# fortio/tray

Measured on AMD Instinct MI355X. Metric: Mrays/sec, seed-2 book-cover scene 1280x720 r=64 d=50; per-pixel L∞ vs ref, higher is better.
Workload: dtype f64; 1 GPU; C2 book-cover seed 2 1280x720 r=64 d=50; traversal=bvh, width=1280, height=720, rays_per_pixel=64, max_depth=50, scene_seed=2, spheres=486, output=float3 f32 linear, parallelism=row-tiles x1, tile_rows=0, frames_in_flight=2, frames_per_launch=16

## Files before the change

tray_amd/csrc/rng.hpp:

```cpp
#pragma once

#include <hip/hip_runtime.h>
#include <stdint.h>

namespace tray {

enum : uint32_t { kPurposeCamera = 1, kPurposeScatter = 3, kPurposeScene = 4, kPurposeKey = 5 };

struct U2 {
    double u0, u1;
};
struct U4 {
    double u0, u1, u2, u3;
};

struct Block {
    uint32_t x0, x1, x2, x3;
};

#ifndef TRAY_PHILOX_ROUNDS
#define TRAY_PHILOX_ROUNDS 10
#endif
__host__ __device__ __forceinline__ Block philox4x32_10(uint64_t seed, uint32_t c0, uint32_t c1, uint32_t c2,
                                                        uint32_t c3) {
    uint32_t k0 = (uint32_t)seed, k1 = (uint32_t)(seed >> 32);
#pragma unroll
    for (int r = 0; r < TRAY_PHILOX_ROUNDS; ++r) {
        if (r > 0) {
            k0 += 0x9E3779B9u;
            k1 += 0xBB67AE85u;
        }
        const uint64_t p0 = (uint64_t)0xD2511F53u * c0;
        const uint64_t p1 = (uint64_t)0xCD9E8D57u * c2;
        const uint32_t n0 = (uint32_t)(p1 >> 32) ^ c1 ^ k0;
        const uint32_t n2 = (uint32_t)(p0 >> 32) ^ c3 ^ k1;
        c0 = n0;
        c1 = (uint32_t)p1;
        c2 = n2;
        c3 = (uint32_t)p0;
    }
    return Block{c0, c1, c2, c3};
}

struct DrawKey {
    uint32_t k0, k1, k2, k3;
};
__host__ __device__ inline DrawKey draw_key(uint64_t seed) {
    const Block b = philox4x32_10(seed, 0u, 0u, 0u, kPurposeKey << 24);
    return DrawKey{b.x0, b.x1, b.x2, b.x3};
}

__host__ __device__ __forceinline__ Block draw_block(uint32_t k0, uint32_t k1, uint32_t k2, uint32_t k3, uint32_t pixel,
                                                     uint32_t sample, uint32_t bounce, uint32_t purpose) {
    uint32_t v0 = (pixel ^ k0) * 1664525u + 1013904223u, v1 = (sample ^ k1) * 1664525u + 1013904223u;
    uint32_t v2 = (bounce ^ k2) * 1664525u + 1013904223u, v3 = (purpose ^ k3) * 1664525u + 1013904223u;
    v0 += v1 * v3;
    v1 += v2 * v0;
    v2 += v0 * v1;
    v3 += v1 * v2;
    v0 ^= v0 >> 16;
    v1 ^= v1 >> 16;
    v2 ^= v2 >> 16;
    v3 ^= v3 >> 16;
    v0 += v1 * v3;
    v1 += v2 * v0;
    v2 += v0 * v1;
    v3 += v1 * v2;
    return Block{v0 ^ (v0 >> 16), v1 ^ (v1 >> 16), v2 ^ (v2 >> 16), v3 ^ (v3 >> 16)};
}

__host__ __device__ __forceinline__ U2 philox_uniforms(uint64_t seed, uint32_t c0, uint32_t c1, uint32_t c2,
                                                       uint32_t c3) {
    const Block b = philox4x32_10(seed, c0, c1, c2, c3);
    const uint64_t a = ((uint64_t)b.x1 << 32) | b.x0;
    const uint64_t c = ((uint64_t)b.x3 << 32) | b.x2;
    U2 u;
    u.u0 = (double)(a >> 11) * 0x1.0p-53;
    u.u1 = (double)(c >> 11) * 0x1.0p-53;
    return u;
}

__host__ __device__ __forceinline__ void sincos_2pi(double u, double& s, double& c) {
    const double v = u * 4.0;
    const double q = __builtin_floor(v);
    const double f = v - q;
    const int quad = (int)q;
    const bool swap = f > 0.5;
    const float x = (float)(swap ? 1.0 - f : f);
    const float t = x * 0x1.921fb6p+0f;
    const float t2 = t * t;
    float sp = __builtin_fmaf(t2, 0x1.71de3ap-19f, -0x1.a01a02p-13f);
    sp = __builtin_fmaf(sp, t2, 0x1.111112p-7f);
    sp = __builtin_fmaf(sp, t2, -0x1.555556p-3f);
    sp = __builtin_fmaf(sp, t2, 1.0f);
    float sn = t * sp;
    float cp = __builtin_fmaf(t2, -0x1.27e4fcp-22f, 0x1.a01a02p-16f);
    cp = __builtin_fmaf(cp, t2, -0x1.6c16c2p-10f);
    cp = __builtin_fmaf(cp, t2, 0x1.555556p-5f);
    cp = __builtin_fmaf(cp, t2, -0.5f);
    float cs = __builtin_fmaf(cp, t2, 1.0f);
    if (swap) {
        const float tmp = sn;
        sn = cs;
        cs = tmp;
    }
    const double sd = sn, cd = cs;
    const double k = 1.5 - 0.5 * (sd * sd + cd * cd);
    const double sk = sd * k, ck = cd * k;
    const int qq = quad & 3;
    s = qq == 0 ? sk : qq == 1 ? ck : qq == 2 ? -sk : -ck;
    c = qq == 0 ? ck : qq == 1 ? -sk : qq == 2 ? -ck : sk;
}

__host__ __device__ __forceinline__ void sincos_2pi_word(uint32_t w, double& s, double& c) {
    const uint32_t F = w & 0x3FFFFFFFu;
    const bool swap = F > 0x20000000u;
    const float x = (float)(swap ? 0x40000000u - F : F) * 0x1p-30f;
    const float t = x * 0x1.921fb6p+0f;
    const float t2 = t * t;
    float sp = __builtin_fmaf(t2, 0x1.71de3ap-19f, -0x1.a01a02p-13f);
    sp = __builtin_fmaf(sp, t2, 0x1.111112p-7f);
    sp = __builtin_fmaf(sp, t2, -0x1.555556p-3f);
    sp = __builtin_fmaf(sp, t2, 1.0f);
    float sn = t * sp;
    float cp = __builtin_fmaf(t2, -0x1.27e4fcp-22f, 0x1.a01a02p-16f);
    cp = __builtin_fmaf(cp, t2, -0x1.6c16c2p-10f);
    cp = __builtin_fmaf(cp, t2, 0x1.555556p-5f);
    cp = __builtin_fmaf(cp, t2, -0.5f);
    float cs = __builtin_fmaf(cp, t2, 1.0f);
    if (swap) {
        const float tmp = sn;
        sn = cs;
        cs = tmp;
    }
    const double sd = sn, cd = cs;
    const double k = 1.5 - 0.5 * (sd * sd + cd * cd);
    const double sk = sd * k, ck = cd * k;
    const uint32_t qq = w >> 30;
    const bool swap_sc = (qq & 1u) != 0u;
    const double s0 = swap_sc ? ck : sk, c0 = swap_sc ? sk : ck;
    const uint64_t sflip = (uint64_t)(qq >> 1) << 63, cflip = (uint64_t)((qq ^ (qq >> 1)) & 1u) << 63;
    s = __builtin_bit_cast(double, __builtin_bit_cast(uint64_t, s0) ^ sflip);
    c = __builtin_bit_cast(double, __builtin_bit_cast(uint64_t, c0) ^ cflip);
}

}
```

tray_amd/csrc/tray_kernel.hip:

```cpp

#include <hip/hip_runtime.h>
#include <stdint.h>
#include <stdlib.h>

#include <algorithm>

#include "bvh.hpp"
#include "fp64.hpp"
#include "rng.hpp"
#include "tray_internal.hpp"
#include "tray_kernel.hpp"

namespace tray {

struct D3 {
    double x, y, z;
};

__device__ __forceinline__ D3 d3(double x, double y, double z) { return D3{x, y, z}; }
__device__ __forceinline__ D3 add(D3 u, D3 v) { return d3(v.x + u.x, v.y + u.y, v.z + u.z); }
__device__ __forceinline__ D3 sub(D3 u, D3 v) { return d3(u.x - v.x, u.y - v.y, u.z - v.z); }
__device__ __forceinline__ D3 smul(D3 v, double t) { return d3(v.x * t, v.y * t, v.z * t); }
__device__ __forceinline__ D3 mul(D3 u, D3 v) { return d3(u.x * v.x, u.y * v.y, u.z * v.z); }
__device__ __forceinline__ D3 sdiv(D3 v, double t) { return d3(v.x / t, v.y / t, v.z / t); }
// ... 532 lines not shown
#define TRAY_WAVE_CHUNKS 32
#endif
#ifndef TRAY_LATE_TAKES
#define TRAY_LATE_TAKES 8u
#endif
__device__ __forceinline__ uint32_t take_chunk(const KernelParams& p, UniPtr uni, uint32_t lane, uint32_t G,
                                               uint32_t& count) {
    typedef __attribute__((address_space(3))) uint64_t LdsU64;
    LdsU64* pool = (LdsU64*)&uni->pool;
    const volatile __attribute__((address_space(3))) uint32_t* pool_end =
        (const volatile __attribute__((address_space(3))) uint32_t*)&uni->pool + 1;
    while (true) {
        uint64_t old = 0;
        if (lane == 0) old = __hip_atomic_fetch_add(pool, (uint64_t)G, __ATOMIC_RELAXED, __HIP_MEMORY_SCOPE_WORKGROUP);
        const uint32_t next = __builtin_amdgcn_readlane((uint32_t)old, 0);
        const uint32_t end = __builtin_amdgcn_readlane((uint32_t)(old >> 32), 0);
        if (end == kPoolDone) return kPoolDone;
        if (next + G <= end) {
            count = G;
            return next;
        }
        if (next <= end) {
            uint32_t base = 0;
            const uint32_t pool_chunks = __builtin_amdgcn_readfirstlane(uni->pool_chunks);
            if (lane == 0) base = atomicAdd(p.queue, pool_chunks);
            base = __builtin_amdgcn_readlane(base, 0);
            const uint64_t fresh = base >= p.nchunks
                                       ? (uint64_t)kPoolDone << 32
                                       : ((uint64_t)min(base + pool_chunks, p.nchunks) << 32) | base;
            if (lane == 0) __hip_atomic_store(pool, fresh, __ATOMIC_RELAXED, __HIP_MEMORY_SCOPE_WORKGROUP);
            if (next < end) {
                count = end - next;
                return next;
            }
            continue;
        }
        while (__builtin_amdgcn_readlane(*pool_end, 0) == end) __builtin_amdgcn_s_sleep(1);
    }
}

__device__ __forceinline__ bool decode_item(const KernelParams& p, uint32_t i, uint32_t tile, int32_t& x, int32_t& j,
                                            uint32_t& s, uint32_t& k) {
    k = 0;
    uint32_t q = udiv(i, p.div_spp, s);
    if (p.passes > 1) q = udiv(q, p.div_passes, k);
    const uint32_t r = q & 63u;
    if (!p.tile_order) tile = q >> 6;
    uint32_t tx;
    const uint32_t ty = udiv(tile, p.div_tiles_x, tx);
    x = (int32_t)(tx * 8u + (r & 7u));
    const int32_t jb = (int32_t)(ty * 8u + (r >> 3));
    j = p.j0 + jb;
    return x < p.width && jb < p.band_rows;
}
__device__ __forceinline__ uint32_t chunk_tile(const KernelParams& p, uint32_t c) {
    if (!p.tile_order) return 0u;
    uint32_t rem;
    return __builtin_amdgcn_readfirstlane(p.tile_order[udiv(c, p.div_chunks_per_tile, rem)]);
}

__device__ __forceinline__ void start_sample(const KernelParams& p, Lane& L, uint32_t item, int32_t x,
                                             int32_t j, uint32_t s) {
    const int32_t y = row_of(p, j);
    L.item = item;
    L.x = x;
    L.j = j;
    L.pixel = (uint32_t)y * (uint32_t)p.width + (uint32_t)x;
    L.sample = s;
    L.bounce = 0;
    L.segments = 0;
    L.thr = d3(1, 1, 1);
    L.busy = true;
    get_ray(p, camera_block(p, L.pixel, s), (double)x, (double)y, L.org, L.dir);
}

template <bool kStats, int kAcc>
__device__ __forceinline__ void end_path(const KernelParams& p, Lane& L, const D3& color, Stats& st,
                                         const AccCtx& acc) {
    if constexpr (kAcc) {
#ifdef TRAY_PROBE_NO_ACC_ADD
        if (color.x != 12345.0) return void(L.busy = false);
#endif
        const uint32_t rs = acc_rshift<kAcc>(p);
        const uint32_t group = ((L.slot << (6u - rs)) | ((L.item & 63u) >> rs));
        LdsF64* s = acc.slabs + (group * kAccCopies + (threadIdx.x % kAccCopies)) * 3u;
        __hip_atomic_fetch_add(s + 0, __builtin_rint(color.x), __ATOMIC_RELAXED, __HIP_MEMORY_SCOPE_WAVEFRONT);
        __hip_atomic_fetch_add(s + 1, __builtin_rint(color.y), __ATOMIC_RELAXED, __HIP_MEMORY_SCOPE_WAVEFRONT);
        __hip_atomic_fetch_add(s + 2, __builtin_rint(color.z), __ATOMIC_RELAXED, __HIP_MEMORY_SCOPE_WAVEFRONT);
#ifdef TRAY_WO_LINEAR_COST
        if (p.tile_cost)
            __hip_atomic_fetch_add(acc.counts + L.slot, L.segments, __ATOMIC_RELAXED, __HIP_MEMORY_SCOPE_WAVEFRONT);
#else
        if (p.tile_cost)
            __hip_atomic_fetch_add(acc.counts + L.slot, L.segments * L.segments, __ATOMIC_RELAXED,
                                   __HIP_MEMORY_SCOPE_WAVEFRONT);
#endif
    } else {
        double* o = p.samples + (size_t)L.item * 3;
        o[0] = color.x;
        o[1] = color.y;
        o[2] = color.z;
    }
    if (p.segments) atomicAdd(p.segments + (size_t)L.j * (size_t)p.width + (size_t)L.x, L.segments);
    if constexpr (kStats) st.segments += L.segments;
    L.busy = false;
}

__device__ __forceinline__ void flush_progress(const KernelParams& p, int32_t t, uint64_t n, uint32_t lane) {
    if (n != 0u && lane == 0u)
        __hip_atomic_fetch_add(p.progress + t, (unsigned long long)n, __ATOMIC_RELAXED, __HIP_MEMORY_SCOPE_SYSTEM);
}
__device__ __forceinline__ void count_progress(const KernelParams& p, bool ended, int32_t j, uint32_t lane,
                                               int32_t& cur, uint64_t& cnt) {
    uint64_t m = __ballot(ended);
    while (m != 0ull) {
        const uint32_t first = (uint32_t)__builtin_ctzll(m);
        const int32_t t0 = __builtin_amdgcn_readlane(j >> 3, first);
        const uint64_t same = __ballot(ended && (j >> 3) == t0) & m;
        if (t0 != cur) {
            flush_progress(p, cur, cnt, lane);
            cur = t0;
            cnt = 0u;
        }
        cnt += (uint64_t)__popcll(same);
        m &= ~same;
    }
}

template <int kFmt>
__device__ __forceinline__ void write_pixel(const KernelParams& p, const double* srgb, D3 mean, int32_t x, int32_t j,
                                            uint32_t pass) {
    const size_t off = (size_t)j * (size_t)p.width + (size_t)x;
    void* const out = static_cast<char*>(p.out) + (size_t)pass * p.out_frame_bytes;
    if constexpr (kFmt == kOutRGBF64) {
        double* o = static_cast<double*>(out) + off * 3;
        o[0] = mean.x;
        o[1] = mean.y;
        o[2] = mean.z;
    } else if constexpr (kFmt == kOutRGBF32) {
        float* o = static_cast<float*>(out) + off * 3;
        o[0] = (float)mean.x;
        o[1] = (float)mean.y;
        o[2] = (float)mean.z;
    } else {
        static_cast<uint32_t*>(out)[off] = srgba_word(srgb, mean.x, mean.y, mean.z);
    }
}
template <int kFmt>
__device__ __forceinline__ void write_mean(const KernelParams& p, const double* srgb, D3 sum, int32_t x, int32_t j,
                                           uint32_t pass) {
    const double inv = 1.0 / (double)p.spp;
    const D3 mean = smul(sum, inv);
    write_pixel<kFmt>(p, srgb, mean, x, j, pass);
}

template <int kAcc>
__device__ __forceinline__ uint64_t acc_retire(const KernelParams& p, const AccCtx& acc, uint64_t open, bool busy,
                                               uint32_t slot, uint32_t chunk_of, uint32_t lane) {
    uint64_t freed = 0;
    while (open != 0ull) {
        const uint32_t s0 = (uint32_t)__builtin_ctzll(open);
        open &= open - 1ull;
        if (__ballot(busy && slot == s0) == 0ull) freed |= 1ull << s0;
    }
    if ((freed >> lane) & 1ull) {
        const uint32_t groups = 64u >> acc_rshift<kAcc>(p);
        uint32_t count = 0u;
        if (p.tile_cost) {
            volatile LdsU32* n = acc.counts;
            count = n[lane];
            n[lane] = 0u;
        }
        for (uint32_t g = 0; g < groups; ++g) {
            const uint32_t slab = kAcc == 1 ? lane : lane * groups + g;
            volatile LdsF64* v = acc.slabs + slab * kAccCopies * 3u;
            double sum[3] = {0.0, 0.0, 0.0};
#pragma unroll
            for (int k = 0; k < kAccCopies; ++k)
#pragma unroll
                for (int c = 0; c < 3; ++c) sum[c] += v[3 * k + c];
#pragma unroll
            for (int k = 0; k < 3 * kAccCopies; ++k) v[k] = 0.0;
            AccPartial* o = reinterpret_cast<AccPartial*>(p.samples) + (kAcc == 1 ? chunk_of : chunk_of * groups + g);
            o->sum[0] = sum[0];
            o->sum[1] = sum[1];
            o->sum[2] = sum[2];
            o->pad = g == 0 ? (double)count : 0.0;
            if constexpr (kAcc == 1) break;
        }
    }
    return freed;
}



template <bool kWild>
__device__ __forceinline__ bool shade_end_color(const KernelParams& p, const Lane& L, bool hit, double dir_lsq,
                                                D3& color) {
    const bool last = L.bounce + 1u >= (uint32_t)p.max_depth;
    const bool blind = kWild ? false : last;
    if (hit && !blind) return true;
    color = d3(0, 0, 0);
    if (!hit) {
        const D3 ud = unit_lsq(L.dir, dir_lsq);
        const double t = 0.5 * (ud.y + 1.0);
        const D3 bg_a = d3(p.bg_a.x, p.bg_a.y, p.bg_a.z), bg_b = d3(p.bg_b.x, p.bg_b.y, p.bg_b.z);
        color = mul(L.thr, add(smul(bg_a, 1.0 - t), smul(bg_b, t)));
    }
    return false;
}
template <bool kStats, int kAcc, bool kWild>
__device__ __forceinline__ bool shade_end(const KernelParams& p, Lane& L, bool hit, double dir_lsq, Stats& st,
                                          const AccCtx& acc) {
    D3 color;
    if (shade_end_color<kWild>(p, L, hit, dir_lsq, color)) return true;
    end_path<kStats, kAcc>(p, L, color, st, acc);
    return false;
}

template <bool kWild, typename GeoAt, typename MatAt>
__device__ __forceinline__ bool shade_scatter_color(const KernelParams& p, Lane& L, double closest, double dir_lsq,
                                                    GeoAt geo_at, MatAt mat_at, D3& color) {
    const double4 g = geo_at();
    const MatRec m = mat_at();
    const Block w = draw(p, L.pixel, L.sample, L.bounce, kPurposeScatter);
    const double u0 = uniform(w.x0);
    D3 ud = d3(0, 0, 0);
    if (m.type != kLambertian) ud = unit_lsq(L.dir, dir_lsq);
    color = d3(0, 0, 0);
    bool ends = false;
    {
        const D3 point = add(L.org, smul(L.dir, closest));
        const D3 outward = sdiv_rcp(sub(point, d3(g.x, g.y, g.z)), m.radius, m.rinv);
        const bool front = dot(L.dir, outward) < 0;
        const D3 normal = neg_if(outward, !front);
        bool scattered = true;
        D3 new_dir;
        D3 att = d3(m.albedo[0], m.albedo[1], m.albedo[2]);
        const bool lambertian = m.type == kLambertian, dielectric = m.type == kDielectric;
        const double cos_theta = go_min1(dot(neg(ud), normal));
        const double z = 1.0 - 2.0 * u0;
        const double sq = sqrt_cr(dielectric ? 1.0 - cos_theta * cos_theta : 1.0 - z * z);
        D3 uv = d3(0, 0, 0);
        if (lambertian || (m.type == kMetal && m.param > 0.0)) uv = unit_vector_from(z, sq, w.x1);
        if (lambertian) {
            new_dir = add(normal, uv);
            if (near_zero(new_dir)) new_dir = normal;
        } else if (m.type == kMetal) {
            D3 reflected = reflect(ud, normal);
            if (m.param > 0.0) reflected = add(reflected, smul(uv, m.param));
            new_dir = reflected;
            scattered = dot(new_dir, normal) > 0;
        } else {
            att = d3(1.0, 1.0, 1.0);
            const double ratio = front ? m.pinv : m.param;
            const double sin_theta = sq;
            const double r0 = front ? m.albedo[0] : m.albedo[1];
            const bool do_reflect = ratio * sin_theta > 1.0 || reflectance(cos_theta, r0) > u0;
            new_dir = do_reflect ? reflect(ud, normal) : refract(ud, normal, ratio);
        }
        if (scattered && (kWild ? L.bounce + 1u < (uint32_t)p.max_depth : true)) {
            L.thr = mul(L.thr, att);
            L.org = point;
            L.dir = new_dir;
            ++L.bounce;
        } else {
            ends = true;
            if constexpr (kWild) color = smul(scattered ? mul(L.thr, att) : L.thr, 0.0);
        }
    }
    __builtin_amdgcn_s_waitcnt(0x0F70);
    return !ends;
}
template <bool kStats, int kAcc, bool kWild, typename GeoAt, typename MatAt>
__device__ __forceinline__ bool shade_scatter(const KernelParams& p, Lane& L, double closest, double dir_lsq,
                                              GeoAt geo_at, MatAt mat_at, Stats& st, const AccCtx& acc) {
    D3 color;
    if (shade_scatter_color<kWild>(p, L, closest, dir_lsq, geo_at, mat_at, color)) return true;
    end_path<kStats, kAcc>(p, L, color, st, acc);
    return false;
}

template <bool kStats, int kAcc, bool kWild, typename GeoAt, typename MatAt>
__device__ __forceinline__ bool shade_step(const KernelParams& p, Lane& L, int best, double closest,
                                           double dir_lsq, GeoAt geo_at, MatAt mat_at, Stats& st, const AccCtx& acc) {
    D3 color;
    bool goes_on = false;
    if (shade_end_color<kWild>(p, L, best >= 0, dir_lsq, color))
        goes_on = shade_scatter_color<kWild>(p, L, closest, dir_lsq, geo_at, mat_at, color);
    if (goes_on) return true;
    end_path<kStats, kAcc>(p, L, color, st, acc);
    return false;
}

#ifndef TRAY_DEVICE_FUNCTIONS_ONLY

#ifndef TRAY_WAVES_PER_SIMD
#define TRAY_WAVES_PER_SIMD 5
#endif
#ifndef TRAY_NODE_STEPS
#define TRAY_NODE_STEPS 3
#endif
#ifndef TRAY_NODE_STEPS_MAX
#define TRAY_NODE_STEPS_MAX 5
#endif
constexpr int kDeepSteps = TRAY_NODE_STEPS_MAX + 1;
// ... 27 lines not shown
            asm volatile("v_add_f32_e64 %0, 1.0, 1.0" : "=v"(t_));            \
        }                                                                     \
    }
#define TRAY_PROBE_F64(n)                                                     \
    {                                                                         \
        _Pragma("unroll") for (int i_ = 0; i_ < (n); ++i_) {                  \
            double t_;                                                        \
            asm volatile("v_add_f64 %0, 1.0, 1.0" : "=v"(t_));                \
        }                                                                     \
    }

#ifdef TRAY_CENSUS
#define TRAY_MARK(name) asm volatile(";@phase " name);
#else
#define TRAY_MARK(name)
#endif

#ifdef TRAY_PROFILE
#define PROF_T0() const uint64_t prof_t0_ = __builtin_amdgcn_s_memtime()
#define PROF_ADD(slot) PROF_CNT(slot, __builtin_amdgcn_s_memtime() - prof_t0_)
#define PROF_CNT(slot, v)                                  \
    {                                                      \
        const unsigned long long v_ = (v);                 \
        if (lane == 0) atomicAdd(prof + (slot), v_);       \
    }
#define PROF_T0E() PROF_T0()
#define PROF_ADDE(slot) PROF_ADD(slot)
#elif defined(TRAY_PROFILE_TIMELINE)
#define PROF_T0() const uint64_t prof_t0_ = (kStats && tl_lone) ? __builtin_amdgcn_s_memtime() : 0
#define PROF_ADD(slot) \
    if (kStats && tl_lone) tl_ph[slot] += __builtin_amdgcn_s_memtime() - prof_t0_
#define PROF_CNT(slot, v)
#else
#define PROF_T0()
#define PROF_ADD(slot)
#define PROF_CNT(slot, v)
#endif
#ifndef TRAY_PROFILE
#define PROF_T0E()
#define PROF_ADDE(slot)
#endif

#if defined(TRAY_PROFILE_BEGIN) && (defined(TRAY_PROFILE_REFILL) || defined(TRAY_PROFILE_CANDWAIT))
#error "TRAY_PROFILE_BEGIN shares profile slots with TRAY_PROFILE_REFILL / TRAY_PROFILE_CANDWAIT"
#endif
#ifdef TRAY_PROFILE_MATERIAL
constexpr int kMatCounters = 26;
__device__ __forceinline__ void prof_material(int site, bool active, int32_t slot, uint32_t bounce, int32_t max_depth,
                                              const MatRec* bmat, uint32_t lane, unsigned long long* pm) {
    int cls = -1;
    if (active) {
        if (slot < 0) cls = 0;
        else if (bounce + 1u >= (uint32_t)max_depth) cls = 1;
        else {
            const MatRec& m = bmat[slot];
            cls = m.type == kLambertian ? 2 : m.type == kDielectric ? 5 : m.param > 0.0 ? 4 : 3;
        }
    }
    unsigned long long* c = pm + site * kMatCounters;
    int bodies = 0;
    for (int k = 0; k < 6; ++k) {
        const uint64_t m = __ballot(cls == k);
        if (lane == 0 && m) {
            atomicAdd(c + k, 1ull);
            atomicAdd(c + 6 + k, (unsigned long long)__popcll(m));
        }
    }
    bodies = (__ballot(cls == 2) ? 1 : 0) + (__ballot(cls == 3 || cls == 4) ? 1 : 0) + (__ballot(cls == 5) ? 1 : 0);
    const int n_di = __popcll(__ballot(cls == 5)), n_me = __popcll(__ballot(cls == 3 || cls == 4));
    const int n_active = __popcll(__ballot(active));
    if (lane == 0) {
        if (n_di) atomicAdd(c + 18 + (n_di >= 8 ? 3 : n_di >= 4 ? 2 : n_di >= 2 ? 1 : 0), 1ull);
        if (n_me) atomicAdd(c + 22 + (n_me >= 8 ? 3 : n_me >= 4 ? 2 : n_me >= 2 ? 1 : 0), 1ull);
        atomicAdd(c + 12 + bodies, 1ull);
        atomicAdd(c + 16, 1ull);
        atomicAdd(c + 17, (unsigned long long)n_active);
    }
}
#define PROF_MATERIAL(site, active) prof_material(site, active, T.slot, L.bounce, p.max_depth, p.bmat, lane, prof_mat)
#else
#define PROF_MATERIAL(site, active)
#endif

#ifdef TRAY_PROFILE_TIMELINE
constexpr uint32_t kTlBuckets = 1024, kTlTicks = 25000, kTlHdr = 6, kTlStride = kTlBuckets + kTlHdr;
#endif

__device__ __forceinline__ uint64_t wave_sum_u64(uint64_t v) {
#pragma unroll
    for (int off = 32; off >= 1; off >>= 1) v += __shfl_xor(v, off, 64);
    return v;
}


__host__ __device__ constexpr size_t bvh_stack_bytes(int32_t slots) { return (size_t)slots * kStackSlotBytes; }

template <int kLDS, bool kBVH, bool kStats, bool kSpill, bool kProg, int kAcc, int kSteps = TRAY_NODE_STEPS_MAX,
          bool kWild = false>
__global__ __launch_bounds__(kBVH ? kBvhBlock : 256, kBVH ? TRAY_BVH_WAVES_PER_SIMD : TRAY_WAVES_PER_SIMD) void render_kernel(KernelParams p) {
    static_assert(!(kWild && (kBVH || kAcc != 0)), "kWild: linear scan, FP64 sums");
    extern __shared__ __attribute__((aligned(16))) double4 smem_all[];
    __attribute__((address_space(3))) Uniforms* uni_lds =
        (__attribute__((address_space(3))) Uniforms*)reinterpret_cast<Uniforms*>(smem_all);
    double4* smem = smem_all + kUniformsBytes / sizeof(double4);
    if (threadIdx.x == 0) {
        volatile __attribute__((address_space(3))) Uniforms* u = uni_lds;
        u->pool = 0;
        u->pool_chunks = p.pool_chunks;
    }
    const UniPtr uni = uni_lds;
    SceneView sv{p.geo,  p.nodes, p.leaves,    p.leaf_single != 0,       p.bgeo, p.bidx,
                 p.bmat, p.n,     p.n_nodes,   p.n_global, p.n_slots - p.n_global};
    Stack<kSpill> S{nullptr, nullptr, 0, 0};
    if constexpr (kBVH) {
        S.base = (__attribute__((address_space(3))) uint32_t*)reinterpret_cast<uint32_t*>(smem) + threadIdx.x;
        S.lds = p.stack_lds;
        S.stride = gridDim.x * blockDim.x;
        if constexpr (kSpill) S.ovf = p.stack_ovf + blockIdx.x * blockDim.x + threadIdx.x;
        double4* scene = smem + bvh_stack_bytes(p.stack_lds) / sizeof(double4);
        if constexpr (kLDS == 1) {
            double4* lds_nodes = scene;
            double4* lds_geo = scene + (size_t)p.n_nodes * (sizeof(Bvh4Node) / sizeof(double4));
            int32_t* lds_idx = reinterpret_cast<int32_t*>(lds_geo + p.n_slots);
            int32_t* lds_leaves = lds_idx + p.n_slots;
            const double4* gn = reinterpret_cast<const double4*>(p.nodes);
            const int n4 = p.n_nodes * (int)(sizeof(Bvh4Node) / sizeof(double4));
            for (int i = threadIdx.x; i < n4; i += blockDim.x) lds_nodes[i] = gn[i];
            for (int i = threadIdx.x; i < p.n_slots; i += blockDim.x) {
                lds_geo[i] = p.bgeo[i];
                lds_idx[i] = p.bidx[i];
            }
            for (int i = threadIdx.x; i < p.n_leaves; i += blockDim.x) lds_leaves[i] = p.leaves[i];
            sv.nodes = reinterpret_cast<const Bvh4Node*>(lds_nodes);
            sv.bgeo = lds_geo;
            sv.bidx = lds_idx;
            sv.leaves = lds_leaves;
        } else if constexpr (kLDS == 2) {
            double4* lds_nodes = scene;
            int32_t* lds_leaves =
                reinterpret_cast<int32_t*>(scene + (size_t)p.n_nodes * (sizeof(Bvh4Node) / sizeof(double4)));
            const double4* gn = reinterpret_cast<const double4*>(p.nodes);
            const int n4 = p.n_nodes * (int)(sizeof(Bvh4Node) / sizeof(double4));
            for (int i = threadIdx.x; i < n4; i += blockDim.x) lds_nodes[i] = gn[i];
            for (int i = threadIdx.x; i < p.n_leaves; i += blockDim.x) lds_leaves[i] = p.leaves[i];
            sv.nodes = reinterpret_cast<const Bvh4Node*>(lds_nodes);
            sv.leaves = lds_leaves;
        }
    } else if constexpr (kLDS == 1) {
        for (int i = threadIdx.x; i < p.n_pad; i += blockDim.x) smem[i] = p.geo[i];
        sv.geo = smem;
    }
    AccCtx acc{nullptr, nullptr};
    uint64_t acc_free = 0;
    uint64_t acc_all = 0;
    uint32_t acc_chunk = 0;
    if constexpr (kAcc) {
        LdsF64* all = (LdsF64*)reinterpret_cast<double*>(reinterpret_cast<char*>(smem_all) + p.acc_off);
        const uint32_t waves = blockDim.x / 64u, slot_f64 = (64u >> acc_rshift<kAcc>(p)) * kAccCopies * 3u;
        const uint32_t slots = (uint32_t)p.acc_slots;
        for (uint32_t i = threadIdx.x; i < waves * slots * slot_f64; i += blockDim.x) all[i] = 0.0;
        acc.slabs = all + (threadIdx.x / 64u) * slots * slot_f64;
        LdsU32* counts = (LdsU32*)(all + waves * slots * slot_f64);
        for (uint32_t i = threadIdx.x; i < waves * slots; i += blockDim.x) counts[i] = 0u;
        acc.counts = counts + (threadIdx.x / 64u) * slots;
        acc_free = acc_all = slots >= 64u ? ~0ull : (1ull << slots) - 1ull;
    }
    __syncthreads();
    const uint32_t lane = threadIdx.x & 63u;
    Lane L;
    L.busy = false;
    Stats st;
    Trav T;
    T.cur = kBvhNone;
    uint32_t pool_next = 0, pool_end = 0;
    uint32_t grp_next = 0, grp_end = 0;

    uint32_t pool_slot = 0;
    uint32_t pool_tile = 0;
    bool exhausted = false;
#ifdef TRAY_STATS_GROUND
    uint32_t gcls = 0;
#endif
    int32_t prog_cur = 0;
    uint64_t prog_cnt = 0;
#ifdef TRAY_PROFILE
    __shared__ unsigned long long prof_lds[16 * 24];
    unsigned long long* prof = prof_lds + 24 * (threadIdx.x / 64u);
    if (lane == 0)
        for (int i = 0; i < 24; ++i) prof[i] = 0;
    const uint64_t prof_start = __builtin_amdgcn_s_memrealtime();
#endif
#ifdef TRAY_PROFILE_MATERIAL
    unsigned long long* prof_mat = p.stats + 32 + 2 * gridDim.x * (blockDim.x / 64u);
#endif
#ifdef TRAY_PROFILE_TIMELINE
    unsigned long long* tl =
        kStats ? p.stats + 32 + (size_t)(blockIdx.x * (blockDim.x / 64u) + threadIdx.x / 64u) * kTlStride : nullptr;
    const uint64_t tl_start = __builtin_amdgcn_s_memrealtime(), tl_mt0 = __builtin_amdgcn_s_memtime();
    uint64_t tl_prev = tl_mt0, tl_acc = 0;
    uint32_t tl_busy = 0, tl_bucket = 0, tl_chunks = 0, tl_dry = 0;
    bool tl_lone = false;
    uint64_t tl_ph[4] = {0, 0, 0, 0};
#endif

    while (true) {
#ifdef TRAY_PROFILE_TIMELINE
        if constexpr (kStats) {
            const uint64_t now = __builtin_amdgcn_s_memtime();
            const uint32_t b = min((uint32_t)((tl_prev - tl_mt0) / kTlTicks), kTlBuckets - 10u);
            if (b != tl_bucket) {
                if (lane == 0) tl[kTlHdr + tl_bucket] = tl_acc;
                tl_bucket = b;
                tl_acc = 0;
            }
            tl_acc += (now - tl_prev) * tl_busy;
            tl_prev = now;
            const uint64_t m = __ballot(L.busy);
            if (exhausted && __popcll(m) == 1) {
                const uint32_t l = (uint32_t)__builtin_ctzll(m);
                const uint32_t seg = __builtin_amdgcn_readlane(L.segments, l);
                const uint32_t pix = __builtin_amdgcn_readlane(L.pixel, l);
                const uint32_t smp = __builtin_amdgcn_readlane(L.sample, l);
                if (lane == 0) {
                    if (!tl_lone) {
                        tl[kTlHdr + kTlBuckets - 5] = now - tl_mt0;
                        tl[kTlHdr + kTlBuckets - 4] = seg;
                    }
                    tl[kTlHdr + kTlBuckets - 3] = seg;
                    tl[kTlHdr + kTlBuckets - 2] = pix;
                    tl[kTlHdr + kTlBuckets - 1] = smp;
                }
                tl_lone = true;
            }
        }
#endif
#if !defined(TRAY_PROFILE_REFILL) && !defined(TRAY_PROFILE_BEGIN)
        PROF_CNT(10, 1);
#endif
        PROF_T0();
        TRAY_MARK("refill_assign")
        uint64_t idle = __ballot(!L.busy);
        if (__popcll(idle) < TRAY_REFILL_BATCH && idle != ~0ull) idle = 0ull;
        uint32_t fresh_item = ~0u, fresh_slot = 0u, fresh_tile = 0u;
        bool cam_hit = false;
#ifdef TRAY_PROFILE_CANDWAIT
        uint64_t prof_wait = 0;
#endif
#ifdef TRAY_PROFILE_REFILL
        uint64_t prof_cam = 0, prof_hit = 0;
#endif
        while (idle != 0ull && !exhausted) {
            if (pool_next == pool_end) {
                if constexpr (kAcc) {
                    if (acc_free == 0ull) {
                        const bool held = L.busy || fresh_item != ~0u;
                        acc_free = acc_retire<kAcc>(kp_fresh(), acc, acc_all, held, L.busy ? L.slot : fresh_slot, acc_chunk,
                                                    lane);
                    }
                    if (acc_free == 0ull) {
                        if (__ballot(L.busy || fresh_item != ~0u) == 0ull) __builtin_trap();
                        break;
                    }
                }
                uint32_t c = grp_next;
                if (grp_next < grp_end) {
                    ++grp_next;
                } else {
                    uint32_t cnt = 1;
                    const KernelParams& pq = kp_fresh();
                    c = take_chunk(pq, uni, lane, grp_end >= pq.late_at ? 1u : pq.wave_chunks, cnt);
                    if (c == kPoolDone) {
                        exhausted = true;
#ifdef TRAY_PROFILE_TIMELINE
                        if constexpr (kStats) tl_dry = (uint32_t)(__builtin_amdgcn_s_memrealtime() - tl_start);
#endif
                        break;
                    }
#ifdef TRAY_PROFILE_TIMELINE
                    tl_chunks += cnt;
#endif
                    grp_next = c + 1;
                    grp_end = c + cnt;
                }
                pool_next = c * 64u;
                pool_end = pool_next + 64u;
                const KernelParams& pc = kp_fresh();
                pool_tile = chunk_tile(pc, c);
                if constexpr (kAcc) {
                    int32_t cx, cj;
                    uint32_t cs, cp;
                    if (acc_rshift<kAcc>(p) < 6u ||
                        (pool_next < pc.items && decode_item(pc, pool_next, pool_tile, cx, cj, cs, cp))) {
                        pool_slot = (uint32_t)__builtin_ctzll(acc_free);
                        acc_free &= ~(1ull << pool_slot);
                        acc_chunk = lane == pool_slot ? c : acc_chunk;
                    }
                }
            }
            const uint32_t n_idle = (uint32_t)__popcll(idle);
            const uint32_t take = min(n_idle, pool_end - pool_next);
            if ((idle >> lane) & 1ull) {
                const uint32_t rank =
                    __builtin_amdgcn_mbcnt_hi((uint32_t)(idle >> 32), __builtin_amdgcn_mbcnt_lo((uint32_t)idle, 0u));
                if (rank < take) {
                    fresh_item = pool_next + rank;
                    fresh_slot = pool_slot;
                    fresh_tile = pool_tile;
                }
            }
            pool_next += take;
            idle = __ballot(!L.busy && fresh_item == ~0u);
        }
#if defined(TRAY_PROFILE) && !defined(TRAY_PROFILE_REFILL)
        {
            const uint64_t fresh = __ballot(fresh_item != ~0u);
            PROF_CNT(13, fresh != 0ull ? 1 : 0);
            PROF_CNT(14, __popcll(fresh));
#ifdef TRAY_PROFILE_BEGIN
            if constexpr (kBVH) PROF_CNT(12, (uint64_t)(fresh != 0ull && __ballot(T.cur == kTravHit) != 0ull) << 40);
#endif
        }
#endif
#ifdef TRAY_PROFILE_REFILL
        const uint64_t prof_assigned = __builtin_amdgcn_s_memtime();
#endif
        if (fresh_item != ~0u) {
            TRAY_MARK("refill_cam")
            const KernelParams& pr = kp_fresh();
            int32_t x, j;
            uint32_t smp, pass;
            if (fresh_item < pr.items && decode_item(pr, fresh_item, fresh_tile, x, j, smp, pass)) {
#ifdef TRAY_PROBE_REFILL
                TRAY_PROBE_F32(TRAY_PROBE_REFILL)
#endif
                uint4 cand = make_uint4(0u, 0u, 0u, kCandOverflow << 16);
                if constexpr (kBVH)
                    if (pr.cand) cand = pr.cand[(size_t)j * (size_t)pr.width + (size_t)x];
                start_sample(pr, L, fresh_item, x, j, (pr.pass0 + pass) * (uint32_t)pr.spp + smp);
                L.slot = fresh_slot;
#ifdef TRAY_PROFILE_REFILL
                prof_cam = __builtin_amdgcn_s_memtime();
#endif
#ifdef TRAY_STATS_GROUND
                gcls = 0;
#endif
#ifdef TRAY_PROFILE_CANDWAIT
                {
                    const uint64_t w0 = __builtin_amdgcn_s_memtime();
                    __builtin_amdgcn_s_waitcnt(0x0F70);
                    prof_wait = __builtin_amdgcn_s_memtime() - w0 + 1u;
                }
#endif
                if constexpr (kBVH) {
                    TRAY_MARK("refill_cand")
                    ++L.segments;
                    T.tlim = __builtin_inff();
                    trav_globals(T, sv, L.org, L.dir);
                    if constexpr (kStats) st.spheres += (uint64_t)sv.n_global;
                    const uint32_t n_cand = cand.w >> 16;
                    const bool listed = n_cand <= kCandSlots;
                    if (listed || !slab_dir_ok(T.a)) {
                        uint64_t lo = ((uint64_t)cand.y << 32) | cand.x, hi = ((uint64_t)cand.w << 32) | cand.z;
                        const uint32_t n_test = listed ? n_cand : (uint32_t)sv.global_first;
#pragma unroll 1
                        for (uint32_t k = 0; k < n_test; ++k) {
                            test_slot(T, sv, listed ? (int32_t)(lo & 0xFFFFu) : (int32_t)k, L.org, L.dir);
                            lo = (lo >> 16) | (hi << 48);
                            hi >>= 16;
                        }
                        if constexpr (kStats) st.spheres += n_test;
                        T.cur = kBvhNone;
                        cam_hit = true;
                    } else {
                        trav_begin32(T, sv, L.org, L.dir);
                    }
                }
#ifdef TRAY_PROFILE_REFILL
                prof_hit = __builtin_amdgcn_s_memtime();
#endif
            }
        }
#ifdef TRAY_PROFILE_REFILL
        const uint64_t prof_shade0 = __builtin_amdgcn_s_memtime();
#endif
        if constexpr (kBVH) {
            if (__ballot(cam_hit) != 0ull) {
                PROF_T0E();
                TRAY_MARK("refill_shade")
                bool ended = false;
                if (cam_hit) {
                    if (shade_end<kStats, kAcc, false>(kp_fresh(), L, T.slot >= 0, T.a, st, acc))
                        T.cur = kTravHitCam;
                    else
                        ended = true;
                }
                if constexpr (kProg) count_progress(p, ended, L.j, lane, prog_cur, prog_cnt);
#ifdef TRAY_PROFILE_BEGIN
                {
                    const uint64_t m = __ballot(T.cur == kTravHitCam);
                    PROF_CNT(11, ((uint64_t)(m != 0ull) << 40) + (uint64_t)__popcll(m));
                }
#endif
                PROF_ADDE(16);
                PROF_CNT(17, 1);
                PROF_CNT(18, __popcll(__ballot(cam_hit)));
            }
        }
#ifdef TRAY_PROFILE_REFILL
        {
            const uint64_t prof_shade1 = __builtin_amdgcn_s_memtime();
            PROF_CNT(10, prof_assigned - prof_t0_);
            PROF_CNT(15, prof_shade1 - prof_shade0);
            const uint64_t mw = __ballot(prof_cam != 0u);
            if (mw != 0ull) {
                const uint32_t lw = (uint32_t)__builtin_ctzll(mw);
                const uint64_t c = ((uint64_t)__builtin_amdgcn_readlane((uint32_t)(prof_cam >> 32), lw) << 32) |
                                   (uint32_t)__builtin_amdgcn_readlane((uint32_t)prof_cam, lw);
                const uint64_t h = ((uint64_t)__builtin_amdgcn_readlane((uint32_t)(prof_hit >> 32), lw) << 32) |
                                   (uint32_t)__builtin_amdgcn_readlane((uint32_t)prof_hit, lw);
                PROF_CNT(13, c - prof_assigned);
                PROF_CNT(14, h - c);
            }
        }
#endif
#ifdef TRAY_PROFILE_CANDWAIT
        {
            const uint64_t mw = __ballot(prof_wait != 0u);
            if (mw != 0ull) {
                const uint32_t lw = (uint32_t)__builtin_ctzll(mw);
                const uint64_t w = ((uint64_t)__builtin_amdgcn_readlane((uint32_t)(prof_wait >> 32), lw) << 32) |
                                   (uint32_t)__builtin_amdgcn_readlane((uint32_t)prof_wait, lw);
                PROF_CNT(15, w - 1u);
            }
        }
#endif
        PROF_ADD(0);
        TRAY_MARK("refill_end")
#ifdef TRAY_PROFILE_TIMELINE
        tl_busy = (uint32_t)__popcll(__ballot(L.busy));
#endif
        if (__ballot(L.busy) == 0ull) {
            if (exhausted) break;
            continue;
        }

        if constexpr (!kBVH) {
            bool ended = false;
            if (L.busy) {
                ++L.segments;
                double closest;
                const int best = scene_hit_linear<TRAY_UNROLL, kStats>(sv, L.org, L.dir, closest, st);
                ended = !shade_step<kStats, kAcc, kWild>(p, L, best, closest, length_sq(L.dir), [&] { return p.geo[max(best, 0)]; },
                                                  [&] { return best >= 0 ? p.mat[best] : MatRec{}; }, st, acc);
            }
            if constexpr (kProg) count_progress(p, ended, L.j, lane, prog_cur, prog_cnt);
        } else {
            if (__ballot(is_marked(T.cur)) != 0ull) {
                PROF_T0();
                TRAY_MARK("scatter_ctl")
                PROF_CNT(20, 1);
                PROF_CNT(21, __popcll(__ballot(is_marked(T.cur))));
#ifdef TRAY_PROFILE_BEGIN
                PROF_CNT(12, __popcll(__ballot(is_marked(T.cur))));
#endif
                PROF_MATERIAL(0, T.cur == kTravHitCam);
                PROF_MATERIAL(1, T.cur == kTravHit);
                bool ended = false;
                if (is_marked(T.cur)) {
                    TRAY_MARK("scatter")
#if defined(TRAY_STATS_GROUND) && !defined(TRAY_PROFILE)
                    const bool from_g = T.slot >= sv.global_first;
#endif
                    if (shade_scatter<kStats, kAcc, false>(kp_fresh(), L, T.closest, T.a, [&] { return sv.bgeo[T.slot]; },
                                                           [&] { return sv.bmat[T.slot]; }, st, acc)) {
                        ++L.segments;
#if defined(TRAY_STATS_GROUND) && !defined(TRAY_PROFILE)
                        {
                            const bool up = L.dir.y >= __builtin_fmax(__builtin_fabs(L.dir.x), __builtin_fabs(L.dir.z));
                            gcls = from_g ? (up ? 1u : 2u) : 0u;
                            if constexpr (kStats) {
                                if (gcls == 1) ++st.g_seg[0];
                                if (gcls != 0) ++st.g_seg[1];
                            }
                        }
#endif
                        T.cur = kTravReady;
                    } else {
                        ended = true;
                        T.cur = kBvhNone;
                    }
                }
                if constexpr (kProg) count_progress(p, ended, L.j, lane, prog_cur, prog_cnt);
                PROF_CNT(22, __popcll(__ballot(ended)));
#ifdef TRAY_PROFILE
                PROF_ADD(19);
#else
                PROF_ADD(3);
#endif
                TRAY_MARK("scatter_end")
            }
            {
                PROF_T0();
#if defined(TRAY_PROFILE) && !defined(TRAY_PROFILE_REFILL) && !defined(TRAY_PROFILE_CANDWAIT)
                PROF_CNT(15, __ballot(T.cur == kTravReady) != 0ull ? 1 : 0);
#endif
                if (T.cur == kTravReady) {
                    TRAY_MARK("begin")
                    trav_begin(T, sv, L.org, L.dir);
                    if constexpr (kStats) st.spheres += (uint64_t)sv.n_global;
                }
#ifdef TRAY_PROFILE
                PROF_ADD(23);
#else
                PROF_ADD(0);
#endif
                TRAY_MARK("begin_end")
            }
            if constexpr (kLDS == 1) {
                if (exhausted) {
                    const KernelParams& pd = kp_fresh();
                    if (pd.coop_lanes != 0u && (uint32_t)__popcll(__ballot(L.busy)) <= pd.coop_lanes) {
                        PROF_T0();
                        uint64_t m = __ballot(L.busy && T.cur != kBvhNone);
                        while (m != 0ull) {
                            const uint32_t l = (uint32_t)__builtin_ctzll(m);
                            m &= m - 1ull;
                            coop_hit(T, sv, pd.n_slots, L.org, L.dir, l, lane);
                        }
                        PROF_ADD(1);
                    }
                }
            }
            {
                PROF_T0();
                TRAY_MARK("node_ctl")
#pragma unroll
                for (int s = 0; s < kSteps; ++s) {
                    const uint64_t m = __ballot(is_trav(T.cur));
                    if (m == 0ull) break;
                    if (s >= TRAY_NODE_STEPS && __popcll(m) < TRAY_NODE_MORE_LANES) break;
                    PROF_CNT(4, 1);
                    PROF_CNT(5, __popcll(m));
#ifndef TRAY_PROFILE_BEGIN
                    PROF_CNT(11, __popcll(__ballot(is_leaf(T.cur))));
                    PROF_CNT(12, __popcll(__ballot(L.busy && T.cur == kBvhNone)));
#endif
                    if (is_trav(T.cur)) {
                        TRAY_MARK("node")
                        uint32_t tested;
#ifdef TRAY_PROBE_NODE
                        TRAY_PROBE_F32(TRAY_PROBE_NODE)
#endif
                        trav_node(T, sv, S, tested);
                        if constexpr (kStats) st.boxes += tested;
#if defined(TRAY_STATS_PRIMARY) && !defined(TRAY_PROFILE)
                        if constexpr (kStats) {
                            ++st.nodes;
                            if (L.bounce == 0) ++st.nodes0, st.boxes0 += tested;
                        }
#endif
#if defined(TRAY_STATS_GROUND) && !defined(TRAY_PROFILE)
                        if constexpr (kStats) {
                            ++st.nodes;
                            if (gcls == 1) ++st.g_nodes[0];
                            if (gcls != 0) ++st.g_nodes[1];
                        }
#endif
                    }
                }
                PROF_ADD(1);
                TRAY_MARK("leaf_decide")
            }
            const uint64_t m_leaf = __ballot(is_leaf(T.cur));
            const uint32_t n_trav = (uint32_t)__popcll(__ballot(is_trav(T.cur)));
            if (m_leaf != 0ull && (__popcll(m_leaf) >= TRAY_LEAF_BATCH || n_trav == 0u ||
                                   (n_trav < TRAY_TRAV_SPARSE && __popcll(m_leaf) >= TRAY_LEAF_LOW))) {
                PROF_T0();
                TRAY_MARK("leaf_ctl")
                PROF_CNT(6, 1);
                PROF_CNT(7, __popcll(m_leaf));
                __builtin_amdgcn_s_setprio(1);
                if (is_leaf(T.cur)) {
                    TRAY_MARK("leaf")
                    uint32_t tested;
#ifdef TRAY_PROBE_LEAF
                    TRAY_PROBE_F32(TRAY_PROBE_LEAF)
#endif
                    trav_leaf(T, sv, S, L.org, L.dir, tested);
                    if constexpr (kStats) st.spheres += tested;
#if defined(TRAY_STATS_PRIMARY) && !defined(TRAY_PROFILE)
                    if constexpr (kStats) {
                        ++st.leaves;
                        if (L.bounce == 0) ++st.leaves0;
                    }
#endif
#if defined(TRAY_STATS_GROUND) && !defined(TRAY_PROFILE)
                    if constexpr (kStats) {
                        ++st.leaves;
                        if (gcls == 1) ++st.g_leaves[0];
                        if (gcls != 0) ++st.g_leaves[1];
                    }
#endif
                }
                PROF_ADD(2);
                __builtin_amdgcn_s_setprio(0);
            }
            const uint64_t m_shade = __ballot(L.busy && T.cur == kBvhNone);
            if (m_shade != 0ull && (__popcll(m_shade) >= TRAY_SHADE_BATCH || __ballot(T.cur < kBvhNone) == 0ull ||
                                    (__popcll(__ballot(is_trav(T.cur))) < TRAY_TRAV_SPARSE &&
                                     __popcll(m_shade) >= TRAY_SHADE_LOW))) {
                PROF_T0();
                TRAY_MARK("shade_ctl")
                PROF_CNT(8, 1);
                PROF_CNT(9, __popcll(m_shade));
                bool ended = false;
                if (L.busy && T.cur == kBvhNone) {
                    TRAY_MARK("shade")
#ifdef TRAY_PROBE_SHADE
                    TRAY_PROBE_F32(TRAY_PROBE_SHADE)
#endif
#ifdef TRAY_PROBE_SHADE64
                    TRAY_PROBE_F64(TRAY_PROBE_SHADE64)
#endif
                    if (shade_end<kStats, kAcc, false>(kp_fresh(), L, T.slot >= 0, T.a, st, acc))
                        T.cur = kTravHit;
                    else
                        ended = true;
                }
                if constexpr (kProg) count_progress(p, ended, L.j, lane, prog_cur, prog_cnt);
#ifdef TRAY_PROFILE_BEGIN
                {
                    const uint64_t m = __ballot(T.cur == kTravHit);
                    PROF_CNT(10, ((uint64_t)(m != 0ull) << 40) + (uint64_t)__popcll(m));
                }
#endif
                PROF_ADD(3);
                TRAY_MARK("shade_end")
            }
        }
    }
    if constexpr (kProg) flush_progress(kp_fresh(), prog_cur, prog_cnt, lane);
    if constexpr (kAcc)
        (void)acc_retire<kAcc>(kp_fresh(), acc, acc_all & ~acc_free, false, 0u, acc_chunk, lane);
    if constexpr (kStats) {
        const uint64_t seg_w = wave_sum_u64(st.segments), sph_w = wave_sum_u64(st.spheres),
                       box_w = wave_sum_u64(st.boxes);
        if (lane == 0) {
            atomicAdd(p.stats + 0, (unsigned long long)seg_w);
            atomicAdd(p.stats + 1, (unsigned long long)sph_w);
            atomicAdd(p.stats + 2, (unsigned long long)box_w);
        }
#if defined(TRAY_STATS_PRIMARY) && !defined(TRAY_PROFILE)
        atomicAdd(p.stats + 3, (unsigned long long)st.nodes0);
        atomicAdd(p.stats + 4, (unsigned long long)st.leaves0);
        atomicAdd(p.stats + 5, (unsigned long long)st.boxes0);
        atomicAdd(p.stats + 6, (unsigned long long)st.nodes);
        atomicAdd(p.stats + 7, (unsigned long long)st.leaves);
#endif
#if defined(TRAY_STATS_GROUND) && !defined(TRAY_PROFILE)
        for (int k = 0; k < 2; ++k) {
            atomicAdd(p.stats + 3 + k, (unsigned long long)st.g_seg[k]);
            atomicAdd(p.stats + 5 + k, (unsigned long long)st.g_nodes[k]);
            atomicAdd(p.stats + 7 + k, (unsigned long long)st.g_leaves[k]);
        }
        atomicAdd(p.stats + 9, (unsigned long long)st.nodes);
        atomicAdd(p.stats + 10, (unsigned long long)st.leaves);
#endif
    }
#ifdef TRAY_PROFILE_TIMELINE
    if (kStats && lane == 0) {
        const uint64_t end = __builtin_amdgcn_s_memrealtime();
        const uint64_t mt_end = __builtin_amdgcn_s_memtime();
        tl_acc += (mt_end - tl_prev) * tl_busy;
        tl[kTlHdr + tl_bucket] = tl_acc;
        for (int k = 0; k < 4; ++k) tl[kTlHdr + kTlBuckets - 9 + k] = tl_ph[k];
        tl[0] = tl_start;
        tl[1] = end;
        tl[2] = tl_dry;
        tl[3] = tl_chunks;
        tl[4] = tl_mt0;
        tl[5] = mt_end;
    }
#endif
#ifdef TRAY_PROFILE
    if (kStats && lane == 0) {
        for (int i = 0; i < 16; ++i) atomicAdd(p.stats + 3 + i, (unsigned long long)prof[i]);
        for (int i = 16; i < 24; ++i) atomicAdd(p.stats + 6 + i, (unsigned long long)prof[i]);
        const uint64_t end = __builtin_amdgcn_s_memrealtime();
        atomicMax(p.stats + 19, (unsigned long long)end);
        atomicAdd(p.stats + 20, (unsigned long long)(end - prof_start));
        atomicMax(p.stats + 21, (unsigned long long)~prof_start);
        const uint32_t wave = blockIdx.x * (blockDim.x / 64u) + threadIdx.x / 64u;
        p.stats[32 + 2 * wave] = prof_start;
        p.stats[33 + 2 * wave] = end;
    }
#endif
}

template <int kFmt>
__device__ __forceinline__ void write_acc_mean(const KernelParams& p, const double* srgb, const int64_t s[3],
                                               uint32_t bad, int32_t x, int32_t j, uint32_t pass) {
    const double unscale = __builtin_ldexp(1.0, -p.acc_shift);
    D3 sum;
    double* c = &sum.x;
#pragma unroll
    for (int k = 0; k < 3; ++k) c[k] = (bad >> k) & 1u ? __builtin_nan("") : (double)s[k] * unscale;
    write_mean<kFmt>(p, srgb, sum, x, j, pass);
}
__device__ __forceinline__ void acc_add(double v, double limit, int64_t& s, uint32_t& bad, int k) {
    if (__builtin_fabs(v) <= limit) s += (int64_t)v;
    else bad |= 1u << k;
}

constexpr int kStageStride = 25;

enum : int { kResolveF64 = 0, kResolveStaged = 1, kResolveFixed = 2, kResolvePartials = 3, kResolveFixedStaged = 4 };
template <int kFmt, int kMode>
__global__ __launch_bounds__(256) void resolve_kernel(KernelParams p) {
    constexpr bool kStaged = kMode == kResolveStaged || kMode == kResolveFixedStaged;
    constexpr bool kFixedStaged = kMode == kResolveFixedStaged;
    __shared__ double srgb[256];
    if constexpr (kFmt == kOutRGBA8) {
        srgb[threadIdx.x] = p.srgb[threadIdx.x];
        __syncthreads();
    }
    const uint32_t q = blockIdx.x * blockDim.x + threadIdx.x;
    if (q == 0 && blockIdx.y == 0) *p.queue = 0u;
    const uint32_t npix = p.frame_items / (uint32_t)p.spp;
    if (q >= npix) return;
    const uint32_t item0 = (q * p.passes + blockIdx.y) * (uint32_t)p.spp;
    const uint32_t pix_stride = p.passes * (uint32_t)p.spp;
    int32_t x, j;
    uint32_t s0, pass;
    const uint32_t tile = p.tile_order ? __builtin_amdgcn_readfirstlane(p.tile_order[q >> 6]) : 0u;
    const bool valid = decode_item(p, item0, tile, x, j, s0, pass);
    D3 sum = d3(0, 0, 0);
    if constexpr (kMode == kResolvePartials) {
        const AccPartial* part = reinterpret_cast<const AccPartial*>(p.samples) + (item0 >> p.acc_rshift);
        if (p.tile_cost) {
            uint64_t n = 0;
            if (valid)
                for (int32_t c = 0; c < (p.spp >> p.acc_rshift); ++c) n += (uint64_t)part[c].pad;
            n = wave_sum_u64(n);
            if ((threadIdx.x & 63u) == 0u)
                atomicAdd(p.tile_cost + (p.tile_order ? tile : q >> 6), (uint32_t)min<uint64_t>(n, 0xFFFFFFFFull));
        }
        if (!valid) return;
        int64_t s[3] = {0, 0, 0};
        uint32_t bad = 0u;
        for (int32_t c = 0; c < (p.spp >> p.acc_rshift); ++c)
#pragma unroll
            for (int k = 0; k < 3; ++k) acc_add(part[c].sum[k], 0x1p53, s[k], bad, k);
        write_acc_mean<kFmt>(p, srgb, s, bad, x, j, pass);
        return;
    } else if constexpr (kMode == kResolveFixed) {
        if (!valid) return;
        const double* smp = p.samples + (size_t)item0 * 3;
        int64_t s[3] = {0, 0, 0};
        uint32_t bad = 0u;
        for (int32_t k = 0; k < p.spp; ++k)
#pragma unroll
            for (int c = 0; c < 3; ++c) acc_add(__builtin_rint(smp[3 * k + c]), 0x1p47, s[c], bad, c);
        write_acc_mean<kFmt>(p, srgb, s, bad, x, j, pass);
        return;
    } else if constexpr (kStaged) {
        __shared__ double stage[4][64 * kStageStride];
        const uint32_t lane = threadIdx.x & 63u;
        double* st = stage[threadIdx.x >> 6];
        const uint32_t q0 = q - lane;
        const double* base = p.samples + ((size_t)q0 * pix_stride + (size_t)blockIdx.y * (uint32_t)p.spp) * 3;
        int64_t si[3] = {0, 0, 0};
        uint32_t bad = 0u;
        for (int32_t s = 0; s < p.spp; s += 8) {
#pragma unroll
            for (int k = 0; k < 12; ++k) {
                const uint32_t t = (uint32_t)k * 64u + lane;
                const uint32_t i = t / 12u, c = t - i * 12u;
                const double2 v = *reinterpret_cast<const double2*>(base + ((size_t)i * pix_stride + s) * 3 + 2 * c);
                st[i * kStageStride + 2 * c] = v.x;
                st[i * kStageStride + 2 * c + 1] = v.y;
            }
            __builtin_amdgcn_fence(__ATOMIC_RELEASE, "wavefront");
            __builtin_amdgcn_wave_barrier();
            __builtin_amdgcn_fence(__ATOMIC_ACQUIRE, "wavefront");
            const double* mine = st + lane * kStageStride;
            if constexpr (kFixedStaged) {
#pragma unroll
                for (int k = 0; k < 24; ++k) acc_add(__builtin_rint(mine[k]), 0x1p47, si[k % 3], bad, k % 3);
            } else {
#pragma unroll
                for (int k = 0; k < 8; ++k) sum = add(sum, d3(mine[3 * k], mine[3 * k + 1], mine[3 * k + 2]));
            }
            __builtin_amdgcn_fence(__ATOMIC_RELEASE, "wavefront");
            __builtin_amdgcn_wave_barrier();
            __builtin_amdgcn_fence(__ATOMIC_ACQUIRE, "wavefront");
        }
// ... 497 lines not shown
```

Before: 13690 Mrays/s.

## Decode pixel once per chunk in accumulate mode and merge sincos swaps

When accumulation runs with one pixel per 64-item chunk, the refill path now decodes pixel coordinates and sample base once per chunk, packing x and the accumulator slot into one register. Each refilled lane then derives its sample index by adding its item id, which removes the per-lane decode_item division work. acc_all is recomputed from the kernel params instead of being held in a live register. Separately, sincos_2pi_word folds the quadrant swap into the reflection swap, so the float values are swapped once instead of swapping the doubles a second time. The changes add compile-time A/B flags, and the chunk-pixel path assumes each chunk maps to a single pixel.

```diff
diff --git a/tray_amd/csrc/rng.hpp b/tray_amd/csrc/rng.hpp
--- a/tray_amd/csrc/rng.hpp
+++ b/tray_amd/csrc/rng.hpp
@@ -114,8 +114,9 @@
 
 __host__ __device__ __forceinline__ void sincos_2pi_word(uint32_t w, double& s, double& c) {
     const uint32_t F = w & 0x3FFFFFFFu;
-    const bool swap = F > 0x20000000u;
-    const float x = (float)(swap ? 0x40000000u - F : F) * 0x1p-30f;
+    const bool reflect = F > 0x20000000u;
+    bool swap = reflect;
+    const float x = (float)(reflect ? 0x40000000u - F : F) * 0x1p-30f;
     const float t = x * 0x1.921fb6p+0f;
     const float t2 = t * t;
     float sp = __builtin_fmaf(t2, 0x1.71de3ap-19f, -0x1.a01a02p-13f);
@@ -128,6 +129,13 @@
     cp = __builtin_fmaf(cp, t2, 0x1.555556p-5f);
     cp = __builtin_fmaf(cp, t2, -0.5f);
     float cs = __builtin_fmaf(cp, t2, 1.0f);
+    const uint32_t qq = w >> 30;
+#ifdef TRAY_AB_SINCOS_TWO_SWAPS
+    const bool swap_sc = (qq & 1u) != 0u;
+#else
+    const bool swap_sc = false;
+    swap = swap != ((qq & 1u) != 0u);
+#endif
     if (swap) {
         const float tmp = sn;
         sn = cs;
@@ -136,8 +144,6 @@
     const double sd = sn, cd = cs;
     const double k = 1.5 - 0.5 * (sd * sd + cd * cd);
     const double sk = sd * k, ck = cd * k;
-    const uint32_t qq = w >> 30;
-    const bool swap_sc = (qq & 1u) != 0u;
     const double s0 = swap_sc ? ck : sk, c0 = swap_sc ? sk : ck;
     const uint64_t sflip = (uint64_t)(qq >> 1) << 63, cflip = (uint64_t)((qq ^ (qq >> 1)) & 1u) << 63;
     s = __builtin_bit_cast(double, __builtin_bit_cast(uint64_t, s0) ^ sflip);
diff --git a/tray_amd/csrc/tray_kernel.hip b/tray_amd/csrc/tray_kernel.hip
--- a/tray_amd/csrc/tray_kernel.hip
+++ b/tray_amd/csrc/tray_kernel.hip
@@ -708,6 +708,11 @@
     const double inv = 1.0 / (double)p.spp;
     const D3 mean = smul(sum, inv);
     write_pixel<kFmt>(p, srgb, mean, x, j, pass);
+}
+
+__device__ __forceinline__ uint64_t acc_all_slots(const KernelParams& p) {
+    const uint32_t slots = (uint32_t)p.acc_slots;
+    return slots >= 64u ? ~0ull : (1ull << slots) - 1ull;
 }
 
 template <int kAcc>
@@ -1041,7 +1046,6 @@
     }
     AccCtx acc{nullptr, nullptr};
     uint64_t acc_free = 0;
-    uint64_t acc_all = 0;
     uint32_t acc_chunk = 0;
     if constexpr (kAcc) {
         LdsF64* all = (LdsF64*)reinterpret_cast<double*>(reinterpret_cast<char*>(smem_all) + p.acc_off);
@@ -1052,7 +1056,7 @@
         LdsU32* counts = (LdsU32*)(all + waves * slots * slot_f64);
         for (uint32_t i = threadIdx.x; i < waves * slots; i += blockDim.x) counts[i] = 0u;
         acc.counts = counts + (threadIdx.x / 64u) * slots;
-        acc_free = acc_all = slots >= 64u ? ~0ull : (1ull << slots) - 1ull;
+        acc_free = acc_all_slots(p);
     }
     __syncthreads();
     const uint32_t lane = threadIdx.x & 63u;
@@ -1066,6 +1070,15 @@
 
     uint32_t pool_slot = 0;
     uint32_t pool_tile = 0;
+#ifdef TRAY_AB_LANE_DECODE
+    constexpr bool kChunkPixel = false;
+#else
+    constexpr bool kChunkPixel = kAcc == 1;
+#endif
+    constexpr uint32_t kXsShift = 24u;
+    static_assert(kAccSlotsMax <= 64, "pool_xs: x | slot << 24 stays non-negative");
+    int32_t pool_xs = -1, pool_j = 0;
+    uint32_t pool_sample = 0;
     bool exhausted = false;
 #ifdef TRAY_STATS_GROUND
     uint32_t gcls = 0;
@@ -1131,6 +1144,8 @@
         uint64_t idle = __ballot(!L.busy);
         if (__popcll(idle) < TRAY_REFILL_BATCH && idle != ~0ull) idle = 0ull;
         uint32_t fresh_item = ~0u, fresh_slot = 0u, fresh_tile = 0u;
+        int32_t fresh_xs = -1, fresh_j = 0;
+        uint32_t fresh_sample = 0u;
         bool cam_hit = false;
 #ifdef TRAY_PROFILE_CANDWAIT
         uint64_t prof_wait = 0;
@@ -1142,9 +1157,10 @@
             if (pool_next == pool_end) {
                 if constexpr (kAcc) {
                     if (acc_free == 0ull) {
-                        const bool held = L.busy || fresh_item != ~0u;
-                        acc_free = acc_retire<kAcc>(kp_fresh(), acc, acc_all, held, L.busy ? L.slot : fresh_slot, acc_chunk,
-                                                    lane);
+                        const bool held = L.busy || (kChunkPixel ? fresh_xs >= 0 : fresh_item != ~0u);
+                        const uint32_t fresh_held = kChunkPixel ? (uint32_t)fresh_xs >> kXsShift : fresh_slot;
+                        acc_free = acc_retire<kAcc>(kp_fresh(), acc, acc_all_slots(kp_fresh()), held,
+                                                    L.busy ? L.slot : fresh_held, acc_chunk, lane);
                     }
                     if (acc_free == 0ull) {
                         if (__ballot(L.busy || fresh_item != ~0u) == 0ull) __builtin_trap();
@@ -1175,7 +1191,18 @@
                 pool_end = pool_next + 64u;
                 const KernelParams& pc = kp_fresh();
                 pool_tile = chunk_tile(pc, c);
-                if constexpr (kAcc) {
+                if constexpr (kChunkPixel) {
+                    int32_t cx;
+                    uint32_t cs, cp;
+                    pool_xs = -1;
+                    if (pool_next < pc.items && decode_item(pc, pool_next, pool_tile, cx, pool_j, cs, cp)) {
+                        pool_sample = (pc.pass0 + cp) * (uint32_t)pc.spp + cs - pool_next;
+                        const uint32_t slot = (uint32_t)__builtin_ctzll(acc_free);
+                        acc_free &= ~(1ull << slot);
+                        acc_chunk = lane == slot ? c : acc_chunk;
+                        pool_xs = cx | (int32_t)(slot << kXsShift);
+                    }
+                } else if constexpr (kAcc) {
                     int32_t cx, cj;
                     uint32_t cs, cp;
                     if (acc_rshift<kAcc>(p) < 6u ||
@@ -1193,8 +1220,14 @@
                     __builtin_amdgcn_mbcnt_hi((uint32_t)(idle >> 32), __builtin_amdgcn_mbcnt_lo((uint32_t)idle, 0u));
                 if (rank < take) {
                     fresh_item = pool_next + rank;
-                    fresh_slot = pool_slot;
-                    fresh_tile = pool_tile;
+                    if constexpr (kChunkPixel) {
+                        fresh_xs = pool_xs;
+                        fresh_j = pool_j;
+                        fresh_sample = pool_sample;
+                    } else {
+                        fresh_slot = pool_slot;
+                        fresh_tile = pool_tile;
+                    }
                 }
             }
             pool_next += take;
@@ -1216,17 +1249,21 @@
         if (fresh_item != ~0u) {
             TRAY_MARK("refill_cam")
             const KernelParams& pr = kp_fresh();
-            int32_t x, j;
-            uint32_t smp, pass;
-            if (fresh_item < pr.items && decode_item(pr, fresh_item, fresh_tile, x, j, smp, pass)) {
+            int32_t x = fresh_xs & (int32_t)((1u << kXsShift) - 1u), j = fresh_j;
+            uint32_t smp = 0, pass = 0;
+            bool valid = fresh_xs >= 0;
+            if constexpr (!kChunkPixel)
+                valid = fresh_item < pr.items && decode_item(pr, fresh_item, fresh_tile, x, j, smp, pass);
+            if (valid) {
 #ifdef TRAY_PROBE_REFILL
                 TRAY_PROBE_F32(TRAY_PROBE_REFILL)
 #endif
                 uint4 cand = make_uint4(0u, 0u, 0u, kCandOverflow << 16);
                 if constexpr (kBVH)
                     if (pr.cand) cand = pr.cand[(size_t)j * (size_t)pr.width + (size_t)x];
-                start_sample(pr, L, fresh_item, x, j, (pr.pass0 + pass) * (uint32_t)pr.spp + smp);
-                L.slot = fresh_slot;
+                start_sample(pr, L, fresh_item, x, j,
+                             kChunkPixel ? fresh_sample + fresh_item : (pr.pass0 + pass) * (uint32_t)pr.spp + smp);
+                L.slot = kChunkPixel ? (uint32_t)fresh_xs >> kXsShift : fresh_slot;
 #ifdef TRAY_PROFILE_REFILL
                 prof_cam = __builtin_amdgcn_s_memtime();
 #endif
@@ -1530,7 +1567,7 @@
     }
     if constexpr (kProg) flush_progress(kp_fresh(), prog_cur, prog_cnt, lane);
     if constexpr (kAcc)
-        (void)acc_retire<kAcc>(kp_fresh(), acc, acc_all & ~acc_free, false, 0u, acc_chunk, lane);
+        (void)acc_retire<kAcc>(kp_fresh(), acc, acc_all_slots(kp_fresh()) & ~acc_free, false, 0u, acc_chunk, lane);
     if constexpr (kStats) {
         const uint64_t seg_w = wave_sum_u64(st.segments), sph_w = wave_sum_u64(st.spheres),
                        box_w = wave_sum_u64(st.boxes);
```

New measurement: 13910 Mrays/s, median of 6. 1.02x the previous value.
